# arkworks-rs/snark

Hardware: AMD Instinct MI355X
Metric: R1CS constraints/sec (Groth16 prove, BLS12-381; throughput: 4 proofs in flight per GPU, z resident in HBM) (higher is better)
Workload: dtype u32

## Files before the change

### snark_amd/csrc/hd.h

```cpp
#pragma once
#if defined(ARK_EMUL)
#include "hip_emul.h"
#define ARK_HD inline
#define ARK_HD_NOINLINE __attribute__((noinline))
#define ARK_D inline
#define ARK_LAUNCH(kernel, grid, block, smem, stream, ...) \
  emu::launch((grid), (block), (smem), [&]() { kernel(__VA_ARGS__); })
#define ARK_DYN_SMEM(T, name) T* name = reinterpret_cast<T*>(emu::g_dyn_smem)
static inline uint32_t ark_pair_xchg(uint32_t v) { return __emu_pair_xchg(v); }
#elif defined(__HIPCC__)
#include <hip/hip_runtime.h>
#define ARK_HD __host__ __device__ __forceinline__
#define ARK_HD_NOINLINE __host__ __device__ __noinline__
#define ARK_D __device__ __forceinline__
#define ARK_LAUNCH(kernel, grid, block, smem, stream, ...) \
  hipLaunchKernelGGL(kernel, (grid), (block), (smem), (stream), __VA_ARGS__)
#define ARK_DYN_SMEM(T, name)                                  \
  extern __shared__ __align__(16) unsigned char _ark_smem[];   \
  T* name = reinterpret_cast<T*>(_ark_smem)
__device__ __forceinline__ uint32_t ark_pair_xchg(uint32_t v) {
#if defined(__HIP_DEVICE_COMPILE__)
  return (uint32_t)__builtin_amdgcn_update_dpp(0, (int)v, 0xB1, 0xF, 0xF, true);
#else
  return v;
#endif
}
#else
#define ARK_HD inline
#define ARK_HD_NOINLINE __attribute__((noinline))
#define ARK_D inline
#endif
```

### snark_amd/csrc/msm28_impl.cuh

```cuda
#pragma once
#include "field28.cuh"
#include "curve.cuh"

namespace ark355 {

template <class P>
struct alignas(16) Affine28 {
  using F = Fp28<P>;
  static constexpr int NB = F::NB;
  static constexpr int WORDS = 2 * NB;
  static constexpr int Q = WORDS / 4;
  static_assert(WORDS % 4 == 0, "row must be a multiple of 16 bytes");
  uint32_t w[WORDS];
  ARK_HD static F unpack(const uint32_t* c) {
    F r;
#pragma unroll
    for (int i = 0; i < F::N; i++) {
      const int bit = 28 * i, q = bit / 32, sh = bit % 32;
      uint32_t v = 0;
      if (q < NB) {
        v = c[q] >> sh;
        if (sh + 28 > 32 && q + 1 < NB) v |= c[q + 1] << (32 - sh);
      }
      r.l[i] = v & F::MASK;
    }
    return r;
  }
  ARK_HD static void pack(const F& a, uint32_t* c) {
#pragma unroll
    for (int q = 0; q < NB; q++) c[q] = 0;
#pragma unroll
    for (int i = 0; i < F::N; i++) {
      const int bit = 28 * i, q = bit / 32, sh = bit % 32;
      if (q < NB) c[q] |= a.l[i] << sh;
      if (sh + 28 > 32 && q + 1 < NB) c[q + 1] |= a.l[i] >> (32 - sh);
    }
  }
};

template <class P>
struct alignas(16) Affine28U {
  using F = Fp28<P>;
  static constexpr int USED = 2 * F::N;
  static constexpr int WORDS = (USED * 4 > 96) ? 32 : ((USED + 3) / 4) * 4;
  static constexpr int Q = USED / 4;
  static_assert(USED % 4 == 0, "limb count must be even");
  uint32_t w[WORDS];
};

#define ARK_KEY_NONE 0xFFFFFFFFu

template <class P>
struct Acc28 {
  Fp28<P> x, y, zz, zzz;
};

template <class P>
struct alignas(16) Slot28 {
  static constexpr int N = Fp28<P>::N;
  static constexpr int WORDS = 4 * N;
  static_assert(WORDS % 4 == 0, "slot must be a whole number of 16-byte words");
  uint32_t w[WORDS];
};
template <class P>
struct alignas(16) Slot28G2 {
  Slot28<P> half[2];
};
template <class P, int COORDS>
using Msm28Slot = typename std::conditional<COORDS == 4, Slot28<P>, Slot28G2<P>>::type;

template <class P>
ARK_HD void slot28_put(Slot28<P>* dst, const Acc28<P>& a, bool empty) {
  constexpr int N = Fp28<P>::N;
  uint4* d = reinterpret_cast<uint4*>(dst);
  uint32_t v[4 * N];
#pragma unroll
  for (int i = 0; i < N; i++) {
    v[0 * N + i] = empty ? 0u : a.x.l[i];
    v[1 * N + i] = empty ? 0u : a.y.l[i];
    v[2 * N + i] = empty ? 0u : a.zz.l[i];
    v[3 * N + i] = empty ? 0u : a.zzz.l[i];
  }
#pragma unroll
  for (int k = 0; k < N; k++) d[k] = make_uint4(v[4 * k], v[4 * k + 1], v[4 * k + 2], v[4 * k + 3]);
}
template <class P>
ARK_HD bool slot28_get(const Slot28<P>* src, Acc28<P>& a) {
  constexpr int N = Fp28<P>::N;
  const uint4* s = reinterpret_cast<const uint4*>(src);
  uint32_t v[4 * N];
#pragma unroll
  for (int k = 0; k < N; k++) {
    const uint4 t = s[k];
    v[4 * k] = t.x;
    v[4 * k + 1] = t.y;
    v[4 * k + 2] = t.z;
    v[4 * k + 3] = t.w;
  }
  uint32_t any = 0;
#pragma unroll
  for (int i = 0; i < N; i++) {
    a.x.l[i] = v[0 * N + i];
    a.y.l[i] = v[1 * N + i];
    a.zz.l[i] = v[2 * N + i];
    a.zzz.l[i] = v[3 * N + i];
    any |= v[2 * N + i];
  }
  return any == 0;
}

template <class P>
ARK_D void msm_flush_slot28(Slot28<P>* buckets_half, Slot28<P>* head_half, Slot28<P>* tail_half, uint32_t* head_key,
                            uint32_t* tail_key, bool write_key, uint32_t key, const Acc28<P>& acc, bool empty, bool first_run,
                            uint32_t run_start, uint32_t run_end, uint32_t seg, const uint32_t* offsets, const uint32_t* counts,
                            size_t slot_stride) {
  const uint32_t o = offsets[key], cnt = counts[key];
  const bool complete = (run_start == o) && (run_end == o + cnt);
  if (complete) {
    slot28_put<P>(reinterpret_cast<Slot28<P>*>(reinterpret_cast<uint8_t*>(buckets_half) + (size_t)key * slot_stride), acc, empty);
  } else if (first_run) {
    slot28_put<P>(reinterpret_cast<Slot28<P>*>(reinterpret_cast<uint8_t*>(head_half) + (size_t)seg * slot_stride), acc, empty);
    if (write_key) head_key[seg] = key;
  } else {
    slot28_put<P>(reinterpret_cast<Slot28<P>*>(reinterpret_cast<uint8_t*>(tail_half) + (size_t)seg * slot_stride), acc, empty);
    if (write_key) tail_key[seg] = key;
  }
}

template <class P, bool PACKED>
using Row28 = typename std::conditional<PACKED, Affine28<P>, Affine28U<P>>::type;

template <class P, bool PACKED>
__global__ void __launch_bounds__(256)
table_to28_kernel(const Affine<Fp<P>>* __restrict__ src, Row28<P, PACKED>* __restrict__ dst, uint64_t rows) {
  using F = Fp28<P>;
  using Row = Row28<P, PACKED>;
  const uint64_t i = (uint64_t)blockIdx.x * blockDim.x + threadIdx.x;
  if (i >= rows) return;
  const Affine<Fp<P>> a = src[i];
  Row o;
#pragma unroll
  for (int k = 0; k < Row::WORDS; k++) o.w[k] = 0;
  if (!a.is_inf()) {
    const F x = F::from_fp(a.x), y = F::from_fp(a.y);
    if constexpr (PACKED) {
      Affine28<P>::pack(x, o.w);
      Affine28<P>::pack(y, o.w + Affine28<P>::NB);
    } else {
#pragma unroll
      for (int k = 0; k < F::N; k++) {
        o.w[k] = x.l[k];
        o.w[F::N + k] = y.l[k];
      }
    }
  }
  dst[i] = o;
}

template <class P>
ARK_HD_NOINLINE int madd28_classify(Fp28<P> pd, Fp28<P> r) {
  if (!Fp28<P>::is_zero_mod_p(pd)) return 0;
  return Fp28<P>::is_zero_mod_p(r) ? 1 : 2;
}
template <class P>
ARK_HD_NOINLINE typename Fp28<P>::Vec dbl28_coord_ni(Fp28<P> px, Fp28<P> py, int which) {
  using F = Fp28<P>;
  const Affine<Fp<P>> a{F::to_fp(px), F::to_fp(py)};
  const XYZZ<Fp<P>> d = xyzz_dbl_affine_t<true>(a);
  return F::from_fp(which == 0 ? d.x : which == 1 ? d.y : which == 2 ? d.zz : d.zzz).to_vec();
}
template <class P>
ARK_HD_NOINLINE typename Fp28<P>::Vec one28_ni() {
  return Fp28<P>::from_fp(Fp<P>::one()).to_vec();
}

template <class P>
struct ZzRegs {
  Acc28<P>& a;
  ARK_D Fp28<P> zz() const { return a.zz; }
  ARK_D Fp28<P> zzz() const { return a.zzz; }
  ARK_D Fp28<P> x() const { return a.x; }
  ARK_D Fp28<P> y() const { return a.y; }
  ARK_D void set_y(const Fp28<P>& v) const { a.y = v; }
  ARK_D void set_zz(const Fp28<P>& v) const { a.zz = v; }
  ARK_D void set_zzz(const Fp28<P>& v) const { a.zzz = v; }
  ARK_D void set_x(const Fp28<P>& v) const { a.x = v; }
};
#ifndef ARK_G2L28_LDS_VALUES
#define ARK_G2L28_LDS_VALUES 4
#endif
template <class P, int NV = ARK_G2L28_LDS_VALUES>
struct ZzLds {
  using F = Fp28<P>;
  static constexpr int N = F::N, QN = (N + 3) / 4;
  static constexpr int VALUES = NV < 2 ? 2 : NV;
  Acc28<P>& a;
  uint4* mine;
  uint32_t stride;
  static size_t bytes(uint32_t threads) { return (size_t)VALUES * QN * threads * sizeof(uint4); }
  ARK_D F get(int s) const {
    asm volatile("" ::: "memory");
    F r;
#pragma unroll
    for (int q = 0; q < QN; q++) {
      const uint4 t = mine[(size_t)(s * QN + q) * stride];
      r.l[4 * q] = t.x;
      if (4 * q + 1 < N) r.l[4 * q + 1] = t.y;
      if (4 * q + 2 < N) r.l[4 * q + 2] = t.z;
      if (4 * q + 3 < N) r.l[4 * q + 3] = t.w;
    }
    return r;
  }
  ARK_D void put(int s, const F& v) const {
#pragma unroll
    for (int q = 0; q < QN; q++)
      mine[(size_t)(s * QN + q) * stride] = make_uint4(v.l[4 * q], 4 * q + 1 < N ? v.l[4 * q + 1] : 0u, 4 * q + 2 < N ? v.l[4 * q + 2] : 0u,
                                                         4 * q + 3 < N ? v.l[4 * q + 3] : 0u);
  }
  ARK_D F zz() const { return get(0); }
  ARK_D F zzz() const { return get(1); }
  ARK_D void set_zz(const F& v) const { put(0, v); }
  ARK_D void set_zzz(const F& v) const { put(1, v); }
  ARK_D F x() const {
    if constexpr (VALUES > 2) return get(2);
    else return a.x;
  }
  ARK_D void set_x(const F& v) const {
    if constexpr (VALUES > 2) put(2, v);
    else a.x = v;
  }
  ARK_D F y() const {
    if constexpr (VALUES > 3) return get(3);
    else return a.y;
  }
  ARK_D void set_y(const F& v) const {
    if constexpr (VALUES > 3) put(3, v);
    else a.y = v;
  }
};

template <class P, class Z>
ARK_D void madd28z(Acc28<P>& acc, const Z& z, bool& empty, const Fp28<P>& px, const Fp28<P>& py, bool negate) {
  using F = Fp28<P>;
  F pys;
  {
    const F n = F::template neg<2, 1>(py);
#pragma unroll
    for (int i = 0; i < F::N; i++) pys.l[i] = negate ? n.l[i] : py.l[i];
  }
  if (empty) {
    const F one = F::from_vec(one28_ni<P>());
    z.set_x(px);
    z.set_y(F::norm(pys));
    z.set_zz(one);
    z.set_zzz(one);
    empty = false;
    return;
  }
  const F U2 = F::mul(px, z.zz());
  const F S2 = F::mul(pys, z.zzz());
  const F Pd = F::template sub<8, 1>(U2, z.x());
  const F R = F::template sub<3, 1>(S2, z.y());
  if (Pd.multiple_hint() < 10u) {
    const int cls = madd28_classify<P>(Pd, R);
    if (cls == 1) {
      const F yn = F::norm(pys);
      z.set_x(F::from_vec(dbl28_coord_ni<P>(px, yn, 0)));
      z.set_y(F::from_vec(dbl28_coord_ni<P>(px, yn, 1)));
      const F nzz = F::from_vec(dbl28_coord_ni<P>(px, yn, 2));
      z.set_zz(nzz);
      z.set_zzz(F::from_vec(dbl28_coord_ni<P>(px, yn, 3)));
      if (nzz.limbs_all_zero()) empty = true;
      return;
    }
    if (cls == 2) {
      empty = true;
      return;
    }
  }
  const F PP = F::sqr(Pd);
  const F PPP = F::mul(Pd, PP);
  const F Q = F::mul(z.x(), PP);
  z.set_zz(F::mul(z.zz(), PP));
  z.set_zzz(F::mul(z.zzz(), PPP));
  const F W = F::add(PPP, F::add(Q, Q));
  const F X3 = F::norm(F::add(F::sqr(R), F::template neg<5, 4>(W)));
  const F T = F::template sub<8, 1>(Q, X3);
  const F NY = F::template neg<3, 1>(z.y());
  z.set_x(X3);
  z.set_y(F::mul2sum(R, T, NY, PPP));
}
template <class P>
ARK_D void madd28(Acc28<P>& acc, bool& empty, const Fp28<P>& px, const Fp28<P>& py, bool negate) {
  const ZzRegs<P> z{acc};
  madd28z<P, ZzRegs<P>>(acc, z, empty, px, py, negate);
}

template <class P>
__global__ void __launch_bounds__(MSM_THREADS)
msm_accumulate28_kernel(const Affine28U<P>* __restrict__ bases, const uint32_t* __restrict__ sorted_keys,
                        const uint32_t* __restrict__ sorted_vals, const uint32_t* __restrict__ total_ptr,
                        const uint32_t* __restrict__ offsets, const uint32_t* __restrict__ counts,
                        Msm28Slot<P, 4>* __restrict__ buckets, Msm28Slot<P, 4>* __restrict__ head,
                        uint32_t* __restrict__ head_key, Msm28Slot<P, 4>* __restrict__ tail,
                        uint32_t* __restrict__ tail_key, uint32_t seg_len) {
  using F = Fp28<P>;
  using Row = Affine28U<P>;
  constexpr int Q = Row::Q;
  const uint32_t seg = blockIdx.x * blockDim.x + threadIdx.x;
  const uint32_t total = *total_ptr;
  const uint64_t start64 = (uint64_t)seg * seg_len;
  if (start64 >= total) return;
  const uint32_t start = (uint32_t)start64;
  const uint32_t end = (start + seg_len < total) ? start + seg_len : total;
  uint32_t cur_key = sorted_keys[start];
  uint32_t run_start = start;
  bool first_run = true;
  bool empty = true;
  Acc28<P> acc;
  acc.x = F::zero();
  acc.y = F::zero();
  acc.zz = F::zero();
  acc.zzz = F::zero();
  auto flush = [&](uint32_t key, uint32_t run_end) __attribute__((always_inline)) {
    msm_flush_slot28<P>(buckets, head, tail, head_key, tail_key, true, key, acc, empty, first_run, run_start, run_end, seg, offsets,
                        counts, sizeof(Slot28<P>));
  };
  uint4 nx[Q];
  uint32_t v_next = sorted_vals[start];
  {
    const uint4* src = reinterpret_cast<const uint4*>(bases + (v_next & ARK_TBL_MASK));
#pragma unroll
    for (int k = 0; k < Q; k++) nx[k] = src[k];
  }
  for (uint32_t e = start; e < end; e++) {
    const uint32_t key = sorted_keys[e];
    const uint32_t v = v_next;
    uint32_t d[4 * Q];
#pragma unroll
    for (int k = 0; k < Q; k++) {
      d[4 * k + 0] = nx[k].x;
      d[4 * k + 1] = nx[k].y;
      d[4 * k + 2] = nx[k].z;
      d[4 * k + 3] = nx[k].w;
    }
    const uint32_t en = (e + 1 < end) ? e + 1 : e;
    v_next = sorted_vals[en];
    {
      const uint4* src = reinterpret_cast<const uint4*>(bases + (v_next & ARK_TBL_MASK));
#pragma unroll
      for (int k = 0; k < Q; k++) nx[k] = src[k];
    }
    if (key != cur_key) {
      flush(cur_key, e);
      cur_key = key;
      run_start = e;
      first_run = false;
      empty = true;
    }
    F px, py;
#pragma unroll
    for (int k = 0; k < F::N; k++) {
      px.l[k] = d[k];
      py.l[k] = d[F::N + k];
    }
    uint32_t any = 0;
#pragma unroll
    for (int k = 0; k < F::N; k++) any |= px.l[k] | py.l[k];
    if (any == 0) continue;
    madd28<P>(acc, empty, px, py, (v >> 31) != 0);
  }
  flush(cur_key, end);
}


template <class P>
struct Park28 {
  using F = Fp28<P>;
  static constexpr int WORDS = 4 * F::N + 4;
  ARK_D static void store(uint32_t* lds, const Acc28<P>& a, bool empty, bool first, uint32_t key, uint32_t start, uint32_t end) {
    uint32_t* d = lds + threadIdx.x;
    if (!empty) {
#pragma unroll
      for (int i = 0; i < F::N; i++) {
        d[(0 * F::N + i) * MSM_THREADS] = a.x.l[i];
        d[(1 * F::N + i) * MSM_THREADS] = a.y.l[i];
        d[(2 * F::N + i) * MSM_THREADS] = a.zz.l[i];
        d[(3 * F::N + i) * MSM_THREADS] = a.zzz.l[i];
      }
    }
    d[(4 * F::N + 0) * MSM_THREADS] = key;
    d[(4 * F::N + 1) * MSM_THREADS] = start;
    d[(4 * F::N + 2) * MSM_THREADS] = end;
    d[(4 * F::N + 3) * MSM_THREADS] = (empty ? 1u : 0u) | (first ? 2u : 0u);
  }
  ARK_D static void load(const uint32_t* lds, Acc28<P>& a, bool& empty, bool& first, uint32_t& key, uint32_t& start, uint32_t& end) {
    const uint32_t* d = lds + threadIdx.x;
    key = d[(4 * F::N + 0) * MSM_THREADS];
    start = d[(4 * F::N + 1) * MSM_THREADS];
    end = d[(4 * F::N + 2) * MSM_THREADS];
    const uint32_t fl = d[(4 * F::N + 3) * MSM_THREADS];
    empty = (fl & 1u) != 0;
    first = (fl & 2u) != 0;
    if (!empty) {
#pragma unroll
      for (int i = 0; i < F::N; i++) {
        a.x.l[i] = d[(0 * F::N + i) * MSM_THREADS];
        a.y.l[i] = d[(1 * F::N + i) * MSM_THREADS];
        a.zz.l[i] = d[(2 * F::N + i) * MSM_THREADS];
        a.zzz.l[i] = d[(3 * F::N + i) * MSM_THREADS];
      }
    }
  }
};

template <class P>
__global__ void __launch_bounds__(MSM_THREADS)
msm_accumulate28p_kernel(const Affine28<P>* __restrict__ bases, const uint32_t* __restrict__ sorted_keys,
                        const uint32_t* __restrict__ sorted_vals, const uint32_t* __restrict__ total_ptr,
                        const uint32_t* __restrict__ offsets, const uint32_t* __restrict__ counts,
                        Msm28Slot<P, 4>* __restrict__ buckets, Msm28Slot<P, 4>* __restrict__ head,
                        uint32_t* __restrict__ head_key, Msm28Slot<P, 4>* __restrict__ tail,
                        uint32_t* __restrict__ tail_key, uint32_t seg_len) {
  using F = Fp28<P>;
  using Row = Affine28<P>;
  constexpr int Q = Row::Q;
  __shared__ uint32_t park_lds[Park28<P>::WORDS * MSM_THREADS];
  const uint32_t seg = blockIdx.x * blockDim.x + threadIdx.x;
  const uint32_t total = *total_ptr;
  const uint64_t start64 = (uint64_t)seg * seg_len;
  if (start64 >= total) return;
  const uint32_t start = (uint32_t)start64;
  const uint32_t end = (start + seg_len < total) ? start + seg_len : total;
  const uint32_t last = end - 1;
  uint32_t cur_key = sorted_keys[start];
  uint32_t run_start = start, run_end = end;
  bool first_run = true;
  bool empty = true;
  Acc28<P> acc;
  acc.x = F::zero();
  acc.y = F::zero();
  acc.zz = F::zero();
  acc.zzz = F::zero();
  bool parked = false;
  auto flush = [&]() __attribute__((always_inline)) {
    msm_flush_slot28<P>(buckets, head, tail, head_key, tail_key, true, cur_key, acc, empty, first_run, run_start, run_end, seg,
                        offsets, counts, sizeof(Slot28<P>));
  };
  uint32_t k0 = cur_key;
  uint32_t v0 = sorted_vals[start];
  uint32_t v1 = sorted_vals[start < last ? start + 1 : last];
  uint4 nx[Q];
  {
    const uint4* src = reinterpret_cast<const uint4*>(bases + (v0 & ARK_TBL_MASK));
#pragma unroll
    for (int k = 0; k < Q; k++) nx[k] = src[k];
  }
  for (uint32_t e = start; e < end; e++) {
    const uint32_t key = k0;
    const uint32_t v = v0;
    uint32_t d[4 * Q];
#pragma unroll
    for (int k = 0; k < Q; k++) {
      d[4 * k + 0] = nx[k].x;
      d[4 * k + 1] = nx[k].y;
      d[4 * k + 2] = nx[k].z;
      d[4 * k + 3] = nx[k].w;
    }
    k0 = sorted_keys[e < last ? e + 1 : last];
    v0 = v1;
    {
      const uint4* src = reinterpret_cast<const uint4*>(bases + (v0 & ARK_TBL_MASK));
#pragma unroll
      for (int k = 0; k < Q; k++) nx[k] = src[k];
    }
    v1 = sorted_vals[e + 2 < end ? e + 2 : last];
    if (key != cur_key) {
      run_end = e;
      if (!parked) {
        Park28<P>::store(park_lds, acc, empty, first_run, cur_key, run_start, e);
        parked = true;
      } else {
        flush();
      }
      cur_key = key;
      run_start = e;
      run_end = end;
      first_run = false;
      empty = true;
    }
    uint32_t any = 0;
#pragma unroll
    for (int k = 0; k < Row::WORDS; k++) any |= d[k];
    if (any == 0) continue;
    const F px = Row::unpack(d), py = Row::unpack(d + Row::NB);
    madd28<P>(acc, empty, px, py, (v >> 31) != 0);
  }
#pragma nounroll
  for (int pass = 0; pass < 2; pass++) {
    flush();
    if (!parked) break;
    Park28<P>::load(park_lds, acc, empty, first_run, cur_key, run_start, run_end);
    parked = false;
  }
}


template <class P, bool PACKED>
struct Affine28G2 {
  Row28<P, PACKED> half[2];
};

template <class P, bool PACKED>
__global__ void __launch_bounds__(256)
table_to28_g2_kernel(const Affine<Fp2<P>>* __restrict__ src, Affine28G2<P, PACKED>* __restrict__ dst, uint64_t rows) {
  using F = Fp28<P>;
  using Row = Row28<P, PACKED>;
  const uint64_t i = (uint64_t)blockIdx.x * blockDim.x + threadIdx.x;
  if (i >= rows) return;
  const Affine<Fp2<P>> a = src[i];
  Affine28G2<P, PACKED> o;
#pragma unroll
  for (int h = 0; h < 2; h++) {
#pragma unroll
    for (int k = 0; k < Row::WORDS; k++) o.half[h].w[k] = 0;
  }
  if (!a.is_inf()) {
    const F x0 = F::from_fp(a.x.c0), x1 = F::from_fp(a.x.c1), y0 = F::from_fp(a.y.c0), y1 = F::from_fp(a.y.c1);
    if constexpr (PACKED) {
      constexpr int NB = Affine28<P>::NB;
      Affine28<P>::pack(x0, o.half[0].w);
      Affine28<P>::pack(y0, o.half[0].w + NB);
      Affine28<P>::pack(x1, o.half[1].w);
      Affine28<P>::pack(y1, o.half[1].w + NB);
    } else {
#pragma unroll
      for (int k = 0; k < F::N; k++) {
        o.half[0].w[k] = x0.l[k];
        o.half[0].w[F::N + k] = y0.l[k];
        o.half[1].w[k] = x1.l[k];
        o.half[1].w[F::N + k] = y1.l[k];
      }
    }
  }
  dst[i] = o;
}

template <class P>
struct Pair28 {
  using F = Fp28<P>;
  static constexpr int N = F::N;
  ARK_D static bool odd() { return (threadIdx.x & 1u) != 0; }
  ARK_D static F xchg(const F& v) {
    F r;
#pragma unroll
    for (int i = 0; i < N; i++) r.l[i] = ark_pair_xchg(v.l[i]);
    return r;
  }
  ARK_D static bool both(bool b) {
    const uint32_t other = ark_pair_xchg(b ? 1u : 0u);
    return b && other != 0;
  }
  ARK_D static F sel(bool c, const F& a, const F& b) {
    F r;
#pragma unroll
    for (int i = 0; i < N; i++) r.l[i] = c ? a.l[i] : b.l[i];
    return r;
  }
  template <uint32_t KA, uint32_t BETA>
  ARK_D static F mul(const F& a, const F& b) {
    const F pa = xchg(a), pb = xchg(b);
    const F npa = F::template neg<KA, BETA>(pa);
    const bool o = odd();
    return F::mul2sum(sel(o, pa, a), b, sel(o, a, npa), pb);
  }
  template <uint32_t KA>
  ARK_D static F sqr(const F& a) {
    const F pa = xchg(a);
    const bool o = odd();
    const F u = F::add(pa, sel(o, pa, a));
    const F d = F::template sub<KA, 1>(a, pa);
    return F::mul(u, sel(o, a, d));
  }
  template <uint32_t KA, uint32_t BA, uint32_t KC, uint32_t BC>
  ARK_D static F mul2(const F& a, const F& b, const F& c, const F& d) {
    const F pa = xchg(a), pb = xchg(b), pc = xchg(c), pd = xchg(d);
    const F npa = F::template neg<KA, BA>(pa), npc = F::template neg<KC, BC>(pc);
    const bool o = odd();
    return F::mul4sum(sel(o, pa, a), b, sel(o, a, npa), pb, sel(o, pc, c), d, sel(o, c, npc), pd);
  }
};

template <class P>
ARK_HD_NOINLINE typename Fp28<P>::Vec dbl28_g2_coord_ni(Fp28<P> x, Fp28<P> y, int which) {
  using F = Fp28<P>;
  using L = Pair28<P>;
  const F U = F::norm(F::add(y, y));
  const F V = L::template sqr<6>(U);
  if (which == 2) return V.to_vec();
  const F W = L::template mul<6, 1>(U, V);
  if (which == 3) return W.to_vec();
  const F S = L::template mul<2, 1>(x, V);
  const F X2 = L::template sqr<3>(x);
  const F M = F::norm(F::add(X2, F::add(X2, X2)));
  const F X3 = F::norm(F::add(L::template sqr<5>(M), F::template neg<4, 2>(F::add(S, S))));
  if (which == 0) return X3.to_vec();
  const F T = F::norm(F::template sub<8, 1>(S, X3));
  const F NW = F::template neg<3, 1>(W);
  return L::template mul2<5, 1, 4, 3>(M, T, NW, y).to_vec();
}

template <class P, class Z>
ARK_D bool madd28_g2_head(Acc28<P>& acc, const Z& z, bool& empty, const Fp28<P>& px, const Fp28<P>& py, bool negate,
                          Fp28<P>& Pd, Fp28<P>& R) {
  using F = Fp28<P>;
  using L = Pair28<P>;
  const F pys = L::sel(negate, F::template neg<2, 1>(py), py);
  if (empty) {
    const F one = L::odd() ? F::zero() : F::from_vec(one28_ni<P>());
    z.set_x(px);
    z.set_y(F::norm(pys));
    z.set_zz(one);
    z.set_zzz(one);
    empty = false;
    return false;
  }
  const F U2 = L::template mul<2, 1>(px, z.zz());
  const F S2 = L::template mul<3, 3>(pys, z.zzz());
  Pd = F::norm(F::template sub<8, 1>(U2, z.x()));
  R = F::norm(F::template sub<3, 1>(S2, z.y()));
  if (L::both(Pd.multiple_hint() < 10u)) {
    if (L::both(F::is_zero_mod_p_inl(Pd))) {
      if (L::both(F::is_zero_mod_p_inl(R))) {
        const F yn = F::norm(pys);
        z.set_x(F::from_vec(dbl28_g2_coord_ni<P>(px, yn, 0)));
        z.set_y(F::from_vec(dbl28_g2_coord_ni<P>(px, yn, 1)));
        const F nzz = F::from_vec(dbl28_g2_coord_ni<P>(px, yn, 2));
        z.set_zz(nzz);
        z.set_zzz(F::from_vec(dbl28_g2_coord_ni<P>(px, yn, 3)));
        if (L::both(nzz.limbs_all_zero())) empty = true;
      } else {
        empty = true;
      }
      return false;
    }
  }
  return true;
}
template <class P, class Z>
ARK_D void madd28_g2_tail(Acc28<P>& acc, const Z& z, const Fp28<P>& Pd, const Fp28<P>& R) {
  using F = Fp28<P>;
  using L = Pair28<P>;
  const F PP = L::template sqr<11>(Pd);
  const F PPP = L::template mul<11, 1>(Pd, PP);
  const F Q = L::template mul<8, 1>(z.x(), PP);
  z.set_zz(L::template mul<3, 1>(z.zz(), PP));
  z.set_zzz(L::template mul<3, 1>(z.zzz(), PPP));
  const F W = F::add(PPP, F::add(Q, Q));
  const F X3 = F::norm(F::add(L::template sqr<6>(R), F::template neg<5, 4>(W)));
  const F T = F::norm(F::template sub<8, 1>(Q, X3));
  const F NY = F::template neg<3, 1>(z.y());
  z.set_x(X3);
  z.set_y(L::template mul2<6, 1, 4, 3>(R, T, NY, PPP));
}
template <class P, class Z>
ARK_D void madd28_g2z(Acc28<P>& acc, const Z& z, bool& empty, const Fp28<P>& px, const Fp28<P>& py, bool negate) {
  Fp28<P> Pd, R;
  if (madd28_g2_head<P, Z>(acc, z, empty, px, py, negate, Pd, R)) madd28_g2_tail<P, Z>(acc, z, Pd, R);
}
template <class P>
ARK_D void madd28_g2(Acc28<P>& acc, bool& empty, const Fp28<P>& px, const Fp28<P>& py, bool negate) {
  const ZzRegs<P> z{acc};
  madd28_g2z<P, ZzRegs<P>>(acc, z, empty, px, py, negate);
}

#ifndef ARK_G2L28_WAVES
#define ARK_G2L28_WAVES 2
#endif
template <class P>
constexpr bool g2l28_zz_in_lds() { return ARK_G2L28_LDS_VALUES > 0 && Fp28<P>::N > 12; }
template <class P, bool ZLDS>
__global__ void __launch_bounds__(MSM_THREADS, ARK_G2L28_WAVES)
msm_accumulate_g2l28_kernel(const Affine28G2<P, false>* __restrict__ bases, const uint32_t* __restrict__ sorted_keys,
                            const uint32_t* __restrict__ sorted_vals, const uint32_t* __restrict__ total_ptr,
                            const uint32_t* __restrict__ offsets, const uint32_t* __restrict__ counts,
                            Msm28Slot<P, 8>* __restrict__ buckets, Msm28Slot<P, 8>* __restrict__ head,
                            uint32_t* __restrict__ head_key, Msm28Slot<P, 8>* __restrict__ tail,
                            uint32_t* __restrict__ tail_key, uint32_t seg_len) {
  using F = Fp28<P>;
  using Zt = typename std::conditional<ZLDS, ZzLds<P>, ZzRegs<P>>::type;
  constexpr int Q = Affine28U<P>::Q;
  const uint32_t gid = blockIdx.x * blockDim.x + threadIdx.x;
  const uint32_t seg = gid >> 1, par = gid & 1u;
  const uint32_t total = *total_ptr;
  const uint64_t start64 = (uint64_t)seg * seg_len;
  if (start64 >= total) return;
  const uint32_t start = (uint32_t)start64;
  const uint32_t end = (start + seg_len < total) ? start + seg_len : total;
  uint32_t cur_key = sorted_keys[start];
  uint32_t run_start = start;
  bool first_run = true;
  bool empty = true;
  Acc28<P> acc;
  acc.x = F::zero();
  acc.y = F::zero();
  acc.zz = F::zero();
  acc.zzz = F::zero();
  ARK_DYN_SMEM(uint4, zlds);
  Zt z = [&]() {
    if constexpr (ZLDS) return ZzLds<P>{acc, zlds + threadIdx.x, blockDim.x};
    else return ZzRegs<P>{acc};
  }();
  auto flush = [&](uint32_t key, uint32_t run_end) __attribute__((always_inline)) {
    if constexpr (ZLDS) {
      if (!empty) {
        acc.x = z.x();
        acc.y = z.y();
        acc.zz = z.zz();
        acc.zzz = z.zzz();
      }
    }
    msm_flush_slot28<P>(&buckets->half[par], &head->half[par], &tail->half[par], head_key, tail_key, par == 0, key, acc, empty,
                        first_run, run_start, run_end, seg, offsets, counts, sizeof(Slot28G2<P>));
  };
  for (uint32_t e = start; e < end; e++) {
    const uint32_t key = sorted_keys[e];
    const uint32_t v = sorted_vals[e];
    F px, py;
    {
      const uint4* src = reinterpret_cast<const uint4*>(&bases[v & ARK_TBL_MASK].half[par]);
      uint32_t d[4 * Q];
#pragma unroll
      for (int k = 0; k < Q; k++) {
        const uint4 t = src[k];
        d[4 * k + 0] = t.x;
        d[4 * k + 1] = t.y;
        d[4 * k + 2] = t.z;
        d[4 * k + 3] = t.w;
      }
#pragma unroll
      for (int k = 0; k < F::N; k++) {
        px.l[k] = d[k];
        py.l[k] = d[F::N + k];
      }
    }
    if (key != cur_key) {
      flush(cur_key, e);
      cur_key = key;
      run_start = e;
      first_run = false;
      empty = true;
    }
    uint32_t any = 0;
#pragma unroll
    for (int k = 0; k < F::N; k++) any |= px.l[k] | py.l[k];
    if ((any | ark_pair_xchg(any)) == 0) continue;
    madd28_g2z<P, Zt>(acc, z, empty, px, py, (v >> 31) != 0);
  }
  flush(cur_key, end);
}

template <class P>
__global__ void __launch_bounds__(MSM_THREADS, ARK_G2L28_WAVES)
msm_accumulate_g2l28p_kernel(const Affine28G2<P, true>* __restrict__ bases, const uint32_t* __restrict__ sorted_keys,
                            const uint32_t* __restrict__ sorted_vals, const uint32_t* __restrict__ total_ptr,
                            const uint32_t* __restrict__ offsets, const uint32_t* __restrict__ counts,
                            Msm28Slot<P, 8>* __restrict__ buckets, Msm28Slot<P, 8>* __restrict__ head,
                            uint32_t* __restrict__ head_key, Msm28Slot<P, 8>* __restrict__ tail,
                            uint32_t* __restrict__ tail_key, uint32_t seg_len) {
  using F = Fp28<P>;
  using Row = Affine28<P>;
  constexpr int Q = Row::Q;
  __shared__ uint32_t park_lds[Park28<P>::WORDS * MSM_THREADS];
  const uint32_t gid = blockIdx.x * blockDim.x + threadIdx.x;
  const uint32_t seg = gid >> 1, par = gid & 1u;
  const uint32_t total = *total_ptr;
  const uint64_t start64 = (uint64_t)seg * seg_len;
  if (start64 >= total) return;
  const uint32_t start = (uint32_t)start64;
  const uint32_t end = (start + seg_len < total) ? start + seg_len : total;
  const uint32_t last = end - 1;
  uint32_t cur_key = sorted_keys[start];
  uint32_t run_start = start, run_end = end;
  bool first_run = true;
  bool empty = true;
  Acc28<P> acc;
  acc.x = F::zero();
  acc.y = F::zero();
  acc.zz = F::zero();
  acc.zzz = F::zero();
  bool parked = false;
  auto flush = [&]() __attribute__((always_inline)) {
    msm_flush_slot28<P>(&buckets->half[par], &head->half[par], &tail->half[par], head_key, tail_key, par == 0, cur_key, acc, empty,
                        first_run, run_start, run_end, seg, offsets, counts, sizeof(Slot28G2<P>));
  };
  uint32_t k0 = cur_key;
  uint32_t v0 = sorted_vals[start];
  for (uint32_t e = start; e < end; e++) {
    const uint32_t key = k0;
    const uint32_t v = v0;
    uint32_t d[4 * Q];
    {
      const uint4* src = reinterpret_cast<const uint4*>(&bases[v & ARK_TBL_MASK].half[par]);
#pragma unroll
      for (int k = 0; k < Q; k++) {
        const uint4 t = src[k];
        d[4 * k + 0] = t.x;
        d[4 * k + 1] = t.y;
        d[4 * k + 2] = t.z;
        d[4 * k + 3] = t.w;
      }
    }
    k0 = sorted_keys[e < last ? e + 1 : last];
    v0 = sorted_vals[e < last ? e + 1 : last];
    if (key != cur_key) {
      run_end = e;
      if (!parked) {
        Park28<P>::store(park_lds, acc, empty, first_run, cur_key, run_start, e);
        parked = true;
      } else {
        flush();
      }
      cur_key = key;
      run_start = e;
      run_end = end;
      first_run = false;
      empty = true;
    }
    uint32_t any = 0;
#pragma unroll
    for (int k = 0; k < Row::WORDS; k++) any |= d[k];
    if ((any | ark_pair_xchg(any)) == 0) continue;
    const F px = Row::unpack(d), py = Row::unpack(d + Row::NB);
    madd28_g2<P>(acc, empty, px, py, (v >> 31) != 0);
  }
#pragma nounroll
  for (int pass = 0; pass < 2; pass++) {
    flush();
    if (!parked) break;
    Park28<P>::load(park_lds, acc, empty, first_run, cur_key, run_start, run_end);
    parked = false;
  }
}

}
```

Baseline: 49.64 million.

## Reuse paired Fp2 exchanges and read partner LDS limbs directly in G2 madd

Restructures the paired-lane Fp2 multiply helpers so that a lane's partner value and its broadcast/negated forms are computed once (the Both struct) and reused across several products in the G2 mixed-add. This drops repeated DPP exchanges of PP, PPP, R and similar values. When zz/zzz/x sit in LDS, the partner limbs are now loaded straight from the neighbouring LDS column instead of going through DPP exchanges. The LDS layout also changes to fixed 64-wide wave-local columns. The cost is more live registers and extra LDS reads, and correctness depends on the pair lanes staying in lockstep within a wave.

```diff
diff --git a/snark_amd/csrc/hd.h b/snark_amd/csrc/hd.h
--- a/snark_amd/csrc/hd.h
+++ b/snark_amd/csrc/hd.h
@@ -8,6 +8,17 @@
   emu::launch((grid), (block), (smem), [&]() { kernel(__VA_ARGS__); })
 #define ARK_DYN_SMEM(T, name) T* name = reinterpret_cast<T*>(emu::g_dyn_smem)
 static inline uint32_t ark_pair_xchg(uint32_t v) { return __emu_pair_xchg(v); }
+static inline uint32_t __emu_pair_bcast0(uint32_t v) {
+  const uint32_t other = __emu_pair_xchg(v);
+  return (threadIdx.x & 1u) ? other : v;
+}
+static inline uint32_t __emu_pair_bcast1(uint32_t v) {
+  const uint32_t other = __emu_pair_xchg(v);
+  return (threadIdx.x & 1u) ? v : other;
+}
+static inline uint32_t ark_pair_bcast0(uint32_t v) { return __emu_pair_bcast0(v); }
+static inline uint32_t ark_pair_bcast1(uint32_t v) { return __emu_pair_bcast1(v); }
+static inline void ark_pair_sync() { (void)__emu_pair_xchg(0u); }
 #elif defined(__HIPCC__)
 #include <hip/hip_runtime.h>
 #define ARK_HD __host__ __device__ __forceinline__
@@ -25,6 +36,21 @@
   return v;
 #endif
 }
+__device__ __forceinline__ uint32_t ark_pair_bcast0(uint32_t v) {
+#if defined(__HIP_DEVICE_COMPILE__)
+  return (uint32_t)__builtin_amdgcn_update_dpp(0, (int)v, 0xA0, 0xF, 0xF, true);
+#else
+  return v;
+#endif
+}
+__device__ __forceinline__ uint32_t ark_pair_bcast1(uint32_t v) {
+#if defined(__HIP_DEVICE_COMPILE__)
+  return (uint32_t)__builtin_amdgcn_update_dpp(0, (int)v, 0xF5, 0xF, 0xF, true);
+#else
+  return v;
+#endif
+}
+__device__ __forceinline__ void ark_pair_sync() {}
 #else
 #define ARK_HD inline
 #define ARK_HD_NOINLINE __attribute__((noinline))
diff --git a/snark_amd/csrc/msm28_impl.cuh b/snark_amd/csrc/msm28_impl.cuh
--- a/snark_amd/csrc/msm28_impl.cuh
+++ b/snark_amd/csrc/msm28_impl.cuh
@@ -174,9 +174,21 @@
   return Fp28<P>::from_fp(Fp<P>::one()).to_vec();
 }
 
+
+template <class P>
+ARK_D Fp28<P> pair_xchg28(const Fp28<P>& v) {
+  Fp28<P> r;
+#pragma unroll
+  for (int i = 0; i < Fp28<P>::N; i++) r.l[i] = ark_pair_xchg(v.l[i]);
+  return r;
+}
 template <class P>
 struct ZzRegs {
+  static constexpr bool IN_LDS = false;
   Acc28<P>& a;
+  ARK_D void zz2(Fp28<P>& own, Fp28<P>& par) const { own = a.zz, par = pair_xchg28<P>(a.zz); }
+  ARK_D void zzz2(Fp28<P>& own, Fp28<P>& par) const { own = a.zzz, par = pair_xchg28<P>(a.zzz); }
+  ARK_D void x2(Fp28<P>& own, Fp28<P>& par) const { own = a.x, par = pair_xchg28<P>(a.x); }
   ARK_D Fp28<P> zz() const { return a.zz; }
   ARK_D Fp28<P> zzz() const { return a.zzz; }
   ARK_D Fp28<P> x() const { return a.x; }
@@ -194,16 +206,18 @@
   using F = Fp28<P>;
   static constexpr int N = F::N, QN = (N + 3) / 4;
   static constexpr int VALUES = NV < 2 ? 2 : NV;
+  static constexpr bool IN_LDS = true;
   Acc28<P>& a;
   uint4* mine;
-  uint32_t stride;
-  static size_t bytes(uint32_t threads) { return (size_t)VALUES * QN * threads * sizeof(uint4); }
+  static constexpr uint32_t STRIDE = 64;
+  static size_t bytes(uint32_t threads) { return (size_t)VALUES * QN * ((threads + STRIDE - 1) / STRIDE * STRIDE) * sizeof(uint4); }
+  ARK_D static uint4* column(uint4* lds) { return lds + (threadIdx.x / STRIDE) * (VALUES * QN * STRIDE) + threadIdx.x % STRIDE; }
   ARK_D F get(int s) const {
     asm volatile("" ::: "memory");
     F r;
 #pragma unroll
     for (int q = 0; q < QN; q++) {
-      const uint4 t = mine[(size_t)(s * QN + q) * stride];
+      const uint4 t = mine[(s * QN + q) * STRIDE];
       r.l[4 * q] = t.x;
       if (4 * q + 1 < N) r.l[4 * q + 1] = t.y;
       if (4 * q + 2 < N) r.l[4 * q + 2] = t.z;
@@ -214,8 +228,30 @@
   ARK_D void put(int s, const F& v) const {
 #pragma unroll
     for (int q = 0; q < QN; q++)
-      mine[(size_t)(s * QN + q) * stride] = make_uint4(v.l[4 * q], 4 * q + 1 < N ? v.l[4 * q + 1] : 0u, 4 * q + 2 < N ? v.l[4 * q + 2] : 0u,
+      mine[(s * QN + q) * STRIDE] = make_uint4(v.l[4 * q], 4 * q + 1 < N ? v.l[4 * q + 1] : 0u, 4 * q + 2 < N ? v.l[4 * q + 2] : 0u,
                                                          4 * q + 3 < N ? v.l[4 * q + 3] : 0u);
+  }
+  ARK_D void get2(int s, F& own, F& par) const {
+    ark_pair_sync();
+    asm volatile("" ::: "memory");
+    const uint4* theirs = (threadIdx.x & 1u) ? mine - 1 : mine + 1;
+#pragma unroll
+    for (int q = 0; q < QN; q++) {
+      const uint4 t = mine[(s * QN + q) * STRIDE];
+      const uint4 u = theirs[(s * QN + q) * STRIDE];
+      own.l[4 * q] = t.x, par.l[4 * q] = u.x;
+      if (4 * q + 1 < N) own.l[4 * q + 1] = t.y, par.l[4 * q + 1] = u.y;
+      if (4 * q + 2 < N) own.l[4 * q + 2] = t.z, par.l[4 * q + 2] = u.z;
+      if (4 * q + 3 < N) own.l[4 * q + 3] = t.w, par.l[4 * q + 3] = u.w;
+    }
+    asm volatile("" ::: "memory");
+    ark_pair_sync();
+  }
+  ARK_D void zz2(F& own, F& par) const { get2(0, own, par); }
+  ARK_D void zzz2(F& own, F& par) const { get2(1, own, par); }
+  ARK_D void x2(F& own, F& par) const {
+    if constexpr (VALUES > 2) get2(2, own, par);
+    else own = a.x, par = pair_xchg28<P>(a.x);
   }
   ARK_D F zz() const { return get(0); }
   ARK_D F zzz() const { return get(1); }
@@ -550,11 +586,15 @@
 struct Pair28 {
   using F = Fp28<P>;
   static constexpr int N = F::N;
+  struct Both {
+    F c0, s1;
+  };
   ARK_D static bool odd() { return (threadIdx.x & 1u) != 0; }
-  ARK_D static F xchg(const F& v) {
+  ARK_D static F xchg(const F& v) { return pair_xchg28<P>(v); }
+  ARK_D static F bcast0(const F& v) {
     F r;
 #pragma unroll
-    for (int i = 0; i < N; i++) r.l[i] = ark_pair_xchg(v.l[i]);
+    for (int i = 0; i < N; i++) r.l[i] = ark_pair_bcast0(v.l[i]);
     return r;
   }
   ARK_D static bool both(bool b) {
@@ -568,26 +608,35 @@
     return r;
   }
   template <uint32_t KA, uint32_t BETA>
+  ARK_D static Both both_of(const F& a) {
+    const F pn = xchg(F::template neg<KA, BETA>(a));
+    return Both{bcast0(a), sel(odd(), a, pn)};
+  }
+  template <uint32_t KA, uint32_t BETA>
+  ARK_D static Both both_with(const F& a, const F& pa) {
+    return Both{bcast0(a), sel(odd(), a, F::template neg<KA, BETA>(pa))};
+  }
+  ARK_D static F mulb(const Both& a, const F& b, const F& pb) { return F::mul2sum(a.c0, b, a.s1, pb); }
+  ARK_D static F mul2b(const Both& a, const F& b, const F& pb, const Both& c, const F& d, const F& pd) {
+    return F::mul4sum(a.c0, b, a.s1, pb, c.c0, d, c.s1, pd);
+  }
+  template <uint32_t KA>
+  ARK_D static F sqr_x(const F& a, const F& pa) {
+    const F u = F::add(bcast0(a), pa);
+    const F d = F::template sub<KA, 1>(a, pa);
+    return F::mul(u, sel(odd(), a, d));
+  }
+  template <uint32_t KA, uint32_t BETA>
   ARK_D static F mul(const F& a, const F& b) {
-    const F pa = xchg(a), pb = xchg(b);
-    const F npa = F::template neg<KA, BETA>(pa);
-    const bool o = odd();
-    return F::mul2sum(sel(o, pa, a), b, sel(o, a, npa), pb);
+    return mulb(both_of<KA, BETA>(a), b, xchg(b));
   }
   template <uint32_t KA>
   ARK_D static F sqr(const F& a) {
-    const F pa = xchg(a);
-    const bool o = odd();
-    const F u = F::add(pa, sel(o, pa, a));
-    const F d = F::template sub<KA, 1>(a, pa);
-    return F::mul(u, sel(o, a, d));
+    return sqr_x<KA>(a, xchg(a));
   }
   template <uint32_t KA, uint32_t BA, uint32_t KC, uint32_t BC>
   ARK_D static F mul2(const F& a, const F& b, const F& c, const F& d) {
-    const F pa = xchg(a), pb = xchg(b), pc = xchg(c), pd = xchg(d);
-    const F npa = F::template neg<KA, BA>(pa), npc = F::template neg<KC, BC>(pc);
-    const bool o = odd();
-    return F::mul4sum(sel(o, pa, a), b, sel(o, a, npa), pb, sel(o, pc, c), d, sel(o, c, npc), pd);
+    return mul2b(both_of<KA, BA>(a), b, xchg(b), both_of<KC, BC>(c), d, xchg(d));
   }
 };
 
@@ -625,8 +674,11 @@
     empty = false;
     return false;
   }
-  const F U2 = L::template mul<2, 1>(px, z.zz());
-  const F S2 = L::template mul<3, 3>(pys, z.zzz());
+  F own, par;
+  z.zz2(own, par);
+  const F U2 = L::mulb(L::template both_of<2, 1>(px), own, par);
+  z.zzz2(own, par);
+  const F S2 = L::mulb(L::template both_of<3, 3>(pys), own, par);
   Pd = F::norm(F::template sub<8, 1>(U2, z.x()));
   R = F::norm(F::template sub<3, 1>(S2, z.y()));
   if (L::both(Pd.multiple_hint() < 10u)) {
@@ -651,17 +703,31 @@
 ARK_D void madd28_g2_tail(Acc28<P>& acc, const Z& z, const Fp28<P>& Pd, const Fp28<P>& R) {
   using F = Fp28<P>;
   using L = Pair28<P>;
-  const F PP = L::template sqr<11>(Pd);
-  const F PPP = L::template mul<11, 1>(Pd, PP);
-  const F Q = L::template mul<8, 1>(z.x(), PP);
-  z.set_zz(L::template mul<3, 1>(z.zz(), PP));
-  z.set_zzz(L::template mul<3, 1>(z.zzz(), PPP));
+  F PPP, own, par;
+  typename L::Both bPP;
+  {
+    const F pPd = L::xchg(Pd);
+    const F PP = L::template sqr_x<11>(Pd, pPd);
+    bPP = L::template both_of<2, 1>(PP);
+    PPP = L::mulb(bPP, Pd, pPd);
+  }
+  const typename L::Both bPPP = L::template both_of<2, 1>(PPP);
+  z.zzz2(own, par);
+  z.set_zzz(L::mulb(bPPP, own, par));
+  z.zz2(own, par);
+  z.set_zz(L::mulb(bPP, own, par));
+  z.x2(own, par);
+  const F Q = L::mulb(bPP, own, par);
   const F W = F::add(PPP, F::add(Q, Q));
-  const F X3 = F::norm(F::add(L::template sqr<6>(R), F::template neg<5, 4>(W)));
+  const F pR = L::xchg(R);
+  const F X3 = F::norm(F::add(L::template sqr_x<6>(R, pR), F::template neg<5, 4>(W)));
   const F T = F::norm(F::template sub<8, 1>(Q, X3));
   const F NY = F::template neg<3, 1>(z.y());
   z.set_x(X3);
-  z.set_y(L::template mul2<6, 1, 4, 3>(R, T, NY, PPP));
+  if constexpr (!Z::IN_LDS && F::N > 12)
+    z.set_y(L::mul2b(L::template both_with<6, 1>(R, pR), T, L::xchg(T), L::template both_of<4, 3>(NY), PPP, L::xchg(PPP)));
+  else
+    z.set_y(L::mul2b(L::template both_with<6, 1>(R, pR), T, L::xchg(T), bPPP, NY, L::xchg(NY)));
 }
 template <class P, class Z>
 ARK_D void madd28_g2z(Acc28<P>& acc, const Z& z, bool& empty, const Fp28<P>& px, const Fp28<P>& py, bool negate) {
@@ -708,7 +774,7 @@
   acc.zzz = F::zero();
   ARK_DYN_SMEM(uint4, zlds);
   Zt z = [&]() {
-    if constexpr (ZLDS) return ZzLds<P>{acc, zlds + threadIdx.x, blockDim.x};
+    if constexpr (ZLDS) return ZzLds<P>{acc, ZzLds<P>::column(zlds)};
     else return ZzRegs<P>{acc};
   }();
   auto flush = [&](uint32_t key, uint32_t run_end) __attribute__((always_inline)) {
```

Measured after the change: 50.20 million, median of 6. 1.1% higher.
